# maxjiang93/space_time_pde

Measured on AMD Instinct MI355X. Metric: query-points/sec (fwd+PDE-residual bwd), rb2d 128^3 latent, higher is better.
Workload: dtype f32; 1 GPU; BASELINE configs[1]: latent [1,32,128,128,32], 2^20 query points, RB2 (3 transport + continuity), ImNet nf=32 softplus, L1 losses, backward to ImNet + UNet3d parameters; points=1048576, parallelism=points sharded x1, unet=UNet3d(igres=(32, 128, 128), nf=16, mf=256) fwd+bwd inside the timed step

## Files before the change

### include/stpde_hip.h

```cpp
#ifndef STPDE_HIP_H
#define STPDE_HIP_H

#ifdef __cplusplus
extern "C" {
#endif

#define STPDE_OK 0
#define STPDE_E_BADARG 1
#define STPDE_E_UNSUPPORTED 2
#define STPDE_E_LAUNCH 3

#define STPDE_ACT_TANH 0
#define STPDE_ACT_RELU 1
#define STPDE_ACT_SOFTPLUS 2
#define STPDE_ACT_ELU 3
#define STPDE_ACT_SWISH 4
#define STPDE_ACT_LEAKYRELU 5

#define STPDE_XT 3
#define STPDE_PBAR_SLOTS 64

typedef struct {
  int S1;
  int S2;
  int pair0[6];
  int pair1[6];
  int act;
  float act_param;
  int combo;
  float alpha[6];
} stpde_jet_cfg;

int stpde_version(void);
int stpde_last_error(char* buf, unsigned long n);
#define STPDE_TUNE_CONV3_LDS_OFF 0
#define STPDE_TUNE_CONV3_LDS_MINBLK 1
#define STPDE_TUNE_CONV3_LDS_GX 2
#define STPDE_TUNE_CONV_WGRAD_LDS_GX 3
#define STPDE_TUNE_CONV1_WGRAD_LDS_GX 4
#define STPDE_TUNE_COUNT 5
int stpde_tune(const char* name, int value);
int stpde_trace_enable(int on);
long stpde_trace_read(char* buf, unsigned long n);

typedef struct {
  int P, N, B, n0, n1, n2, C;
  int p_base;
  float lo_c[3], hi_c[3], cube[3];
  float alpha[6];
} stpde_gather_desc;
int stpde_lig_gather(const stpde_gather_desc* d, const float* pts, const float* latent, float* X, float* XR,
                     float* coef, int* cell, float* cw , void* stream);

typedef struct {
  int ntiles, KT, MT, first_hidden;
  stpde_jet_cfg cfg;
  int mfma_bf16;
  int packed;
  int det;
} stpde_layer_desc;
int stpde_jet_layer_fwd(const stpde_layer_desc* d, const float* in_pre, const float* X, const float* Wh_pack,
                        const float* Ws_pack, const float* tanc, const float* W0s_pack, const float* tanc0,
                        float* out_pre, const float* cw ,
                        const void* Wh_pack_bf16, float* z0, void* stream);

int stpde_jet_tail_fwd(const stpde_jet_cfg* cfg, int ntiles, int nf16, const float* in_pre2, const float* X,
                       const float* const* Wh_pack, const float* const* Ws_pack, const float* const* tanc,
                       float* const* out_pre, const float* cw, void* stream);

int stpde_jet_tail_fwd_p(const stpde_jet_cfg* cfg, int ntiles, int nf16, const float* in_pre2, const float* X,
                         const float* const* Wh_pack, const float* const* Ws_pack, const float* const* tanc,
                         float* const* out_pre, const float* cw, int packed, const void* const* Wh16_pack, void* stream);

int stpde_jet_tail_bwd(const stpde_jet_cfg* cfg, int ntiles, int nf16, const float* abar5, const float* const* WhT_pack,
                       const float* const* pre, float* const* abar_out, const float* cw, float* act_param_bar,
                       void* stream);

int stpde_jet_tail_bwd_p(const stpde_jet_cfg* cfg, int ntiles, int nf16, const float* abar5, const float* const* WhT_pack,
                         const float* const* pre, float* const* abar_out, const float* cw, float* act_param_bar, int packed,
                         const void* const* WhT16_pack, void* stream);

int stpde_jet_layer_bwd(const stpde_layer_desc* d, const float* abar_out, const float* WhT_pack, float* in_pre,
                        const float* X, const float* W0s_pack, const float* tanc0, float* abar0, const float* cw,
                        float* act_param_bar, const void* WhT_pack_bf16 ,
                        float* abar0_tan, const float* z0, void* stream);

int stpde_jet_layer_bwd_to(const stpde_layer_desc* d, const float* abar_out, const float* WhT_pack, const float* in_pre,
                           float* abar_in, const float* cw, float* act_param_bar, const void* WhT_pack_bf16, void* stream);

int stpde_jet_wgrad(const stpde_layer_desc* d, int SP, const float* abar_out, const float* in_pre, const float* X,
                    const float* tanc0, float* dW_aug, const float* cw, void* stream);

int stpde_jet_fc1_bwd_supported(const stpde_layer_desc* d);
int stpde_jet_fc1_bwd(const stpde_layer_desc* d, const float* abar1, const void* WhT_pack_bf16, const float* z0,
                      const float* tanc0, const float* cw, const float* X, float* abar0, float* abar0_tan, float* dW_aug,
                      float* act_param_bar, void* stream);

int stpde_lig_reduce_fwd(const stpde_jet_cfg* cfg, int S_mlp, int P, int n_out, const float* out_pre,
                         const float* coef, float* jets, long ldp, void* stream);
int stpde_lig_reduce_bwd(const stpde_jet_cfg* cfg, int S_mlp, int P, int n_out, const float* jets_bar, long ldp,
                         const float* coef, float* abar_out, void* stream);

int stpde_jet_tan0_reduce(int ntiles, int MT, const float* abar0_tan, float* dW_aug, int ldw, int det ,
                          void* stream);

typedef struct {
  int ntiles, nlayers, C, n1, n2;
  int MT[8];
  int SP[8];
  int packed[8];
  int S[8];
} stpde_xbar_desc;
int stpde_lig_xbar_scatter(const stpde_xbar_desc* d, const float* const* abar, const float* const* WsL_pack,
                           const int* cell, float* dlatent, void* stream);
int stpde_lig_xbar_rows(const stpde_xbar_desc* d, const float* const* abar, const float* const* WsL_pack,
                        float* xrows, void* stream);
int stpde_lig_dlatent_reduce(int B, int n0, int n1, int n2, int C, const float* xrows, const int* perm,
                             const int* start, float* dlatent, void* stream);

typedef struct {
  int nlayers;
  int cin, cout, nf16;
  int KT[8], MT[8];
  const float* Wh[8];
  const float* WhT[8];
  const float* Ws[8];
  const float* WsL[8];
  const float* tanc[8];
  const void* Wh16[8];
  const void* WhT16[8];
  int mfma_bf16;
  int packed_mask;
  long dw_off[8];
} stpde_imnet_plan;
typedef struct {
  float* X;
  float* XR;
  float* coef;
  float* cw;
  int* cell;
  float* pre[8];
  float* abar2x;
  float* abar3x;
  float* tan0;
  float* abar0;
  float* abar1x;
  float* abar0x;
  float* xrows;
  int* perm;
  int* start;
  void* sort_tmp;
  unsigned long sort_tmp_bytes;
  float* abar4x;
} stpde_lig_workspace;
#define STPDE_F_STASH 1
#define STPDE_F_VALUE_TILES 2
#define STPDE_F_FUSED_TAIL 4
#define STPDE_F_TAN0_ROWSUM 8
#define STPDE_F_DETERMINISTIC 16
#define STPDE_F_WGRAD 32
#define STPDE_F_WGRAD_FP32 64
#define STPDE_F_PHASE_A 128
#define STPDE_F_PHASE_B 256
#define STPDE_F_NO_FC1_FUSED 512
#define STPDE_F_DET 1024
int stpde_lig_imnet_jet_fwd(const stpde_imnet_plan* plan, const stpde_jet_cfg* cfg_mlp, const stpde_jet_cfg* cfg_out,
                            const stpde_gather_desc* gd, const float* pts, const float* latent,
                            const stpde_lig_workspace* ws, float* jets, long ldp, int flags, void* stream);
int stpde_lig_imnet_jet_bwd(const stpde_imnet_plan* plan, const stpde_jet_cfg* cfg_mlp, const stpde_jet_cfg* cfg_out,
                            const stpde_jet_cfg* cfg_val, const stpde_gather_desc* gd, const stpde_lig_workspace* ws,
                            const float* jets_bar, long ldp, float* dW_flat, float* dlatent, float* act_param_bar,
                            int flags, void* stream);
unsigned long stpde_lig_sort_tmp_bytes(int P, long n_nodes);
int stpde_lig_cell_sort(int P, long n_nodes, const int* cell, int* perm, int* start, void* tmp, unsigned long tmp_bytes,
                        void* stream);

typedef struct {
  int P, N, B, dim, C;
  int n[4];
  float lo_c[4], hi_c[4], cube[4];
} stpde_interp_desc;
int stpde_interp_fwd(const stpde_interp_desc* d, const float* grid, const float* pts, float* out ,
                     float* corner_values , float* weights ,
                     float* x_relative , void* stream);
int stpde_interp_bwd_grid(const stpde_interp_desc* d, const float* pts, const float* out_bar,
                          const float* corner_bar, float* dgrid, void* stream);

typedef struct {
  int D, P, N, B, C;
  int p_base;
  int ntiles;
  int n[4];
  float lo_c[4], hi_c[4], cube[4];
// ... 222 lines not shown
```

### space_time_pde_amd/csrc/api.cpp

```cpp
#include <hip/hip_runtime.h>

#include <cstdarg>
#include <cstdio>
#include <cstring>
#include <mutex>
#include <set>
#include <string>

#include "../../include/stpde_hip.h"

static thread_local char g_err[512] = "";

void stpde_set_error(const char* fmt, ...) {
  va_list ap;
  va_start(ap, fmt);
  vsnprintf(g_err, sizeof(g_err), fmt, ap);
  va_end(ap);
}

int stpde_check_launch(const char* what) {
  hipError_t e = hipGetLastError();
  if (e != hipSuccess) {
    stpde_set_error("%s: launch failed: %s", what, hipGetErrorString(e));
    return STPDE_E_LAUNCH;
  }
  return STPDE_OK;
}

extern "C" int stpde_version(void) { return 316; }

#include <atomic>
static const char* const g_tune_names[STPDE_TUNE_COUNT] = {"conv3_lds_off", "conv3_lds_minblk", "conv3_lds_gx", "conv_wgrad_lds_gx",
                                                           "conv1_wgrad_lds_gx"};
static std::atomic<int> g_tune[STPDE_TUNE_COUNT];
int stpde_tune_get(int key) { return (key >= 0 && key < STPDE_TUNE_COUNT) ? g_tune[key].load(std::memory_order_relaxed) : 0; }
extern "C" int stpde_tune(const char* name, int value) {
  if (!name) return -1;
  for (int k = 0; k < STPDE_TUNE_COUNT; ++k)
    if (!strcmp(name, g_tune_names[k])) return g_tune[k].exchange(value);
  stpde_set_error("stpde_tune: unknown key '%s'", name);
  return -1;
}

extern "C" int stpde_last_error(char* buf, unsigned long n) {
  if (!buf || n == 0) return STPDE_E_BADARG;
  strncpy(buf, g_err, n - 1);
  buf[n - 1] = 0;
  return STPDE_OK;
}

int stpde_trace_on = 0;
static std::mutex g_trace_mu;
static std::set<std::string> g_trace;

void stpde_trace_note(const char* launcher, const char* kernel) {
  std::lock_guard<std::mutex> lk(g_trace_mu);
  g_trace.insert(std::string(kernel) + " @ " + launcher);
}

extern "C" int stpde_trace_enable(int on) {
  std::lock_guard<std::mutex> lk(g_trace_mu);
  g_trace.clear();
  stpde_trace_on = on ? 1 : 0;
  return STPDE_OK;
}

extern "C" long stpde_trace_read(char* buf, unsigned long n) {
  std::lock_guard<std::mutex> lk(g_trace_mu);
  std::string all;
  for (const auto& s : g_trace) all += s + "\n";
  if (buf && n > 0) {
    strncpy(buf, all.c_str(), n - 1);
    buf[n - 1] = 0;
  }
  return (long)all.size() + 1;
}
```

### space_time_pde_amd/csrc/jet_wgrad_impl.h

```cpp
#pragma once
#include <cstdlib>

#include "common.h"

struct WgradArgs {
  const float* P;
  const float* Q;
  const float* X;
  const float* tanc0;
  float* dW;
  const float* cw;
  int SP, KT, MT, ntiles;
  int gx, gy, gz;
  int kz0;
  int det;
  int bf16;
  int pk;
  int ncoord;
  int xfold;
  stpde_jet_cfg cfg;
};

#ifndef STPDE_QUAD_PIPE
#define STPDE_QUAD_PIPE 1
#endif
#ifndef STPDE_ABLATE_W
#define STPDE_ABLATE_W 0
#endif
#ifndef STPDE_X3_XFOLD
#define STPDE_X3_XFOLD 1
#endif
#ifndef STPDE_WG_RPIPE
#define STPDE_WG_RPIPE 1
#endif
#ifndef STPDE_X3_EARLYP
#define STPDE_X3_EARLYP 0
#endif
template <int TP>
__device__ __forceinline__ void lds_put_T(float* blk, int lane, f32x4 v) {
  const int g = lane >> 4, j = lane & 15;
  float* w = blk + (4 * g) * TP + j;
  w[0] = v[0];
  w[TP] = v[1];
  w[2 * TP] = v[2];
  w[3 * TP] = v[3];
}
template <int TP>
__device__ __forceinline__ void lds_put_R(float* blk, int lane, f32x4 v) {
  *reinterpret_cast<f32x4*>(blk + (lane & 15) * TP + 4 * (lane >> 4)) = v;
}
template <int TP>
__device__ __forceinline__ f32x4 lds_get_R(const float* blk, int lane) {
  return *reinterpret_cast<const f32x4*>(blk + (lane & 15) * TP + 4 * (lane >> 4));
}

template <int S1, int S2, int MODE, int ACT, int KC, bool HASX, bool BF = false, int SPL = 1, int PKM = 0>
__global__ __launch_bounds__(512, 2) void k_wgrad_coop(WgradArgs a) {
  static_assert(SPL == 1 || (BF && SPL == 3), "operand splitting is a bf16-pipe mode");
  constexpr int PMODE = (PKM & 4) ? 2 : 0;
  constexpr int S = 1 + S1 + S2, MCW = 2, NW = 8, RS = 8;
  constexpr int NM = KC;
  constexpr bool SPLP = BF && SPL == 3;
  constexpr int TP = (2 * RS * S * 16 * 24 * 4 + NW * 2 * 16 * 24 * 4 <= 150 * 1024) ? 24 : 20;
  constexpr int TBLK = 16 * TP;
  constexpr int BLK = BF ? 128 * SPL : TBLK;
  constexpr int NBUF = (2 * RS * S * BLK * 4 + NW * 2 * BLK * 4 <= 150 * 1024) ? 2 : 1;
  constexpr int SX = S1 == 3 ? 4 : 1;
  __shared__ __attribute__((aligned(16))) float hl[NBUF][RS][S][BLK];
  constexpr int NPP = (BF && SPL == 1 && 2 * RS * S * 512 + NW * S * MCW * 512 <= 100 * 1024) ? S * MCW : 2;
  __shared__ __attribute__((aligned(16))) float pp[NW][NPP][BLK];
  const int lane = threadIdx.x & 63;
  const int wv = threadIdx.x >> 6;
  const int lo = lane * 4;
  const int KT = a.KT, MT = a.MT, SP = a.SP;
  const int L = blockIdx.x, xcd = L & 7, slot = L >> 3;
  const int kz = (slot % a.gz) + a.kz0, tq = slot / a.gz;
  const int mg = tq % a.gy, bx = (tq / a.gy) * 8 + xcd;
  const int ms = wv % NM, ks = wv / NM;
  const int mt0 = (mg * NM + ms) * MCW;
  const int kq0 = kz * RS;
  const int g = lane >> 4, c = lane & 15;

  f32x4 acc[MCW][KC];
#pragma unroll
  for (int mi = 0; mi < MCW; ++mi)
#pragma unroll
    for (int ki = 0; ki < KC; ++ki) acc[mi][ki] = f32x4{0.f, 0.f, 0.f, 0.f};

  auto put = [&](float* blk, f32x4 v, bool row_major) {
    if constexpr (BF) {
      __bf16* hb16 = reinterpret_cast<__bf16*>(blk);
#pragma unroll
      for (int t = 0; t < SPL; ++t) {
        const bf16x4 h = to_bf4(v);
        *reinterpret_cast<bf16x4*>(hb16 + (t * 16 + (lane & 15)) * 16 + 4 * (lane >> 4)) = h;
        if (t + 1 < SPL) v -= bf4_to_f32(h);
      }
    } else if (row_major) {
      lds_put_R<TP>(blk, lane, v);
    } else {
      lds_put_T<TP>(blk, lane, v);
    }
  };
  auto get = [&](const float* blk) -> f32x4 { return lds_get_R<TP>(blk, lane); };
  auto get16 = [&](const float* blk, int t, bool cm = true) -> bf16x4 {
    const __bf16* b16 = reinterpret_cast<const __bf16*>(blk) + t * 256;
    if (cm) return lds_read_tr16(b16 + (4 * (lane >> 4) + ((lane & 15) >> 2)) * 16 + 4 * (lane & 3));
    return *reinterpret_cast<const bf16x4*>(b16 + (lane & 15) * 16 + 4 * (lane >> 4));
  };

  auto x_rowmajor = [&](f32x4 v) -> f32x4 {
    float* patch = pp[wv][0];
    __builtin_amdgcn_wave_barrier();
    lds_put_T<TP>(patch, lane, v);
    __builtin_amdgcn_wave_barrier();
    const f32x4 r = lds_get_R<TP>(patch, lane);
    __builtin_amdgcn_wave_barrier();
    return r;
  };
  auto x_rowmajor16 = [&](f32x4 v, bf16x4* t) {
    float* patch = pp[wv][0];
    __builtin_amdgcn_wave_barrier();
    put(patch, v, false);
    __builtin_amdgcn_wave_barrier();
#pragma unroll
    for (int k = 0; k < (BF ? SPL : 1); ++k) t[k] = get16(patch, k, true);
    __builtin_amdgcn_wave_barrier();
  };
  auto load_q = [&](int tile, f32x4* pre, float* cq) {
    const int kq = kq0 + wv;
    if (!HASX || kq < KT) {
      load_cq<S2>(a.cw, tile * 2 + (c >> 3), cq);
      if (MODE == 1) {
        pre[0] = ld4(a.Q + ((size_t)tile * KT + kq) * 256 + lo);
        if (S1 == 3) {
#pragma unroll
          for (int d = 0; d < 3; ++d) pre[1 + d] = ld4(a.tanc0 + ((size_t)d * KT + kq) * 256 + lo);
#pragma unroll
          for (int p = 0; p < S2; ++p) pre[4 + p] = f32x4{0.f, 0.f, 0.f, 0.f};
        }
      } else {
#pragma unroll
        for (int st = 0; st < S; ++st) pre[st] = ld_blk(a.Q, (PKM & 1) ? 1 : 0, tile, S, KT, st, kq, lane);
      }
    } else if (kq < KT + XT) {
      pre[0] = ld4(a.X + ((size_t)tile * XT + (kq - KT)) * 256 + lo);
    }
  };
  auto finish_q = [&](const f32x4* pre, const float* cq, int buf) {
    const int kq = kq0 + wv;
    if (!HASX || kq < KT) {
      f32x4 H[S];
      act_jet_fwd<S1, S2, ACT>(a.cfg, pre, H, cq);
#pragma unroll
      for (int st = 0; st < S; ++st) put(&hl[buf][wv][st][0], H[st], false);
    } else if (kq < KT + XT) {
      const int xt = kq - KT;
      put(&hl[buf][wv][0][0], pre[0], false);
      if (S1 == 3) {
#pragma unroll
        for (int d = 0; d < 3; ++d) {
          f32x4 v;
#pragma unroll
          for (int r = 0; r < 4; ++r) v[r] = (xt == 0 && 4 * g + r == d && d < a.ncoord) ? 1.f : 0.f;
          put(&hl[buf][wv][1 + d][0], v, false);
        }
      }
    }
  };
  auto produce = [&](int tile, int buf) {
    f32x4 pre[S];
    float cq[6];
// ... 4 lines not shown
#pragma unroll
    for (int st = 0; st < S; ++st)
#pragma unroll
      for (int mi = 0; mi < MCW; ++mi) {
        const int mt = mt0 + mi < MT ? mt0 + mi : MT - 1;
        raw[st][mi] = st < SP ? ld_blk_raw(a.P, PMODE, tile, SP, MT, st, mt, lane) : f32x4{0.f, 0.f, 0.f, 0.f};
      }
  };
  auto transpose_p = [&](f32x4 (*raw)[MCW], f32x4 (*pa)[MCW]) {
    if constexpr (BF) return;
#pragma unroll
    for (int st = 0; st < S; ++st)
#pragma unroll
      for (int mi = 0; mi < MCW; ++mi) {
        float* patch = pp[wv][(st * MCW + mi) & 1];
        lds_put_T<TP>(patch, lane, blk_val(raw[st][mi], st < SP ? PMODE : 0, st));
        __builtin_amdgcn_wave_barrier();
        pa[st][mi] = lds_get_R<TP>(patch, lane);
        __builtin_amdgcn_wave_barrier();
      }
  };

  constexpr int SH = (S + 1) / 2, SXH = (SX + 1) / 2;
  bf16x8 pa8[BF ? SPL : 1][BF ? SH : 1][MCW];
  const bf16x4 zero4 = to_bf4(f32x4{0.f, 0.f, 0.f, 0.f});
  auto pack_p = [&](f32x4 (*raw_)[MCW]) {
    if constexpr (BF && NPP > 2) {
#pragma unroll
      for (int st = 0; st < S; ++st)
#pragma unroll
        for (int mi = 0; mi < MCW; ++mi) put(pp[wv][st * MCW + mi], blk_val(raw_[st][mi], st < SP ? PMODE : 0, st), false);
      __builtin_amdgcn_wave_barrier();
#pragma unroll
      for (int sp = 0; sp < SH; ++sp)
#pragma unroll
        for (int mi = 0; mi < MCW; ++mi)
          pa8[0][sp][mi] = cat8(get16(pp[wv][2 * sp * MCW + mi], 0, true),
                                2 * sp + 1 < S ? get16(pp[wv][(2 * sp + 1 < S ? 2 * sp + 1 : 0) * MCW + mi], 0, true) : zero4);
      __builtin_amdgcn_wave_barrier();
    } else if constexpr (BF) {
      int flip = 0;
      auto terms = [&](f32x4 v, bf16x4* t) {
        float* patch = pp[wv][flip];
        flip ^= 1;
        put(patch, v, false);
        __builtin_amdgcn_wave_barrier();
#pragma unroll
        for (int k = 0; k < SPL; ++k) t[k] = get16(patch, k, true);
        __builtin_amdgcn_wave_barrier();
      };
#pragma unroll
      for (int sp = 0; sp < SH; ++sp)
#pragma unroll
        for (int mi = 0; mi < MCW; ++mi) {
          bf16x4 t0[SPL], t1[SPL];
          terms(blk_val(raw_[2 * sp][mi], 2 * sp < SP ? PMODE : 0, 2 * sp), t0);
          if (2 * sp + 1 < S) terms(blk_val(raw_[2 * sp + 1][mi], 2 * sp + 1 < SP ? PMODE : 0, 2 * sp + 1), t1);
#pragma unroll
          for (int k = 0; k < SPL; ++k) pa8[k][sp][mi] = cat8(t0[k], 2 * sp + 1 < S ? t1[k] : zero4);
        }
    }
  };
  auto mma16 = [&](f32x4& c, int sp, int mi, const bf16x8* H8) {
    if constexpr (SPL == 3) {
      constexpr int TP[6] = {1, 0, 2, 0, 1, 0}, TH[6] = {1, 2, 0, 1, 0, 0};
#pragma unroll
      for (int q6 = 0; q6 < 6; ++q6) c = mfma_bf(pa8[TP[q6]][sp][mi], H8[TH[q6]], c);
    } else {
      c = mfma_bf(pa8[0][sp][mi], H8[0], c);
    }
  };

  const int stride = a.gx;
  int tile = bx;
  f32x4 pa[S][MCW];
  constexpr bool XF = !HASX && !BF;
  constexpr bool XB = !HASX && BF && SPL == 1;
  constexpr bool XS = !HASX && BF && SPL == 3 && STPDE_X3_XFOLD;
  const int xslot = (kz - a.kz0) * (NW / NM) + ks;
  const int xsel = xslot < XT ? xslot : XT - 1;
  f32x4 accx[(XF || XB || XS) ? MCW : 1];
  float acct[XF && S1 == 3 ? 3 : 1][XF ? MCW : 1];
  const bf16x4 one4 = to_bf4(f32x4{1.f, 1.f, 1.f, 1.f});
  const bool tanw = (XB || XS) && S1 == 3 && xslot == 0;
  const bf16x4 e0 = (tanw && c == 0) ? one4 : zero4;
  const bf16x8 x8t = cat8((tanw && c == 1 && a.ncoord > 1) ? one4 : zero4, (tanw && c == 2 && a.ncoord > 2) ? one4 : zero4);
  f32x4 xr = f32x4{0.f, 0.f, 0.f, 0.f};
  if constexpr (XF || XB || XS) {
#pragma unroll
    for (int mi = 0; mi < MCW; ++mi) accx[mi] = f32x4{0.f, 0.f, 0.f, 0.f};
  }
  if constexpr (XF && S1 == 3) {
#pragma unroll
    for (int d = 0; d < 3; ++d)
#pragma unroll
      for (int mi = 0; mi < MCW; ++mi) acct[d][mi] = 0.f;
  }
  auto xb_mma = [&]() {
    if constexpr (XB) {
      bf16x4 xt1[1];
      x_rowmajor16(xr, xt1);
      const bf16x8 x8 = cat8(xt1[0], S1 == 3 ? e0 : zero4);
#pragma unroll
      for (int mi = 0; mi < MCW; ++mi) accx[mi] = mfma_bf(pa8[0][0][mi], x8, accx[mi]);
      if constexpr (S1 == 3) {
#pragma unroll
        for (int mi = 0; mi < MCW; ++mi) accx[mi] = mfma_bf(pa8[0][1][mi], x8t, accx[mi]);
      }
    }
  };
  auto xs_mma = [&]() {
    if constexpr (XS) {
      bf16x4 xt3[3];
      x_rowmajor16(xr, xt3);
      constexpr int TP[6] = {1, 0, 2, 0, 1, 0}, TH[6] = {1, 2, 0, 1, 0, 0};
#pragma unroll
      for (int q6 = 0; q6 < 6; ++q6) {
        const bf16x8 x8 = cat8(xt3[TH[q6]], (S1 == 3 && TH[q6] == 0) ? e0 : zero4);
#pragma unroll
        for (int mi = 0; mi < MCW; ++mi) accx[mi] = mfma_bf(pa8[TP[q6]][0][mi], x8, accx[mi]);
      }
      if constexpr (S1 == 3) {
#pragma unroll
        for (int k = 2; k >= 0; --k)
#pragma unroll
          for (int mi = 0; mi < MCW; ++mi) accx[mi] = mfma_bf(pa8[k][1][mi], x8t, accx[mi]);
      }
    }
  };
  auto ring_mma = [&](int rb) {
    auto rd = [&](int ki, bf16x8* H8) {
      const int q = ks * KC + ki;
#pragma unroll
      for (int sp = 0; sp < SH; ++sp)
        H8[sp] = cat8(get16(&hl[rb][q][2 * sp][0], 0, true),
                      2 * sp + 1 < S ? get16(&hl[rb][q][2 * sp + 1 < S ? 2 * sp + 1 : 0][0], 0, true) : zero4);
    };
    bf16x8 Hn[SH];
    rd(0, Hn);
#pragma unroll
    for (int ki = 0; ki < KC; ++ki) {
      bf16x8 Hc[SH];
#pragma unroll
      for (int sp = 0; sp < SH; ++sp) Hc[sp] = Hn[sp];
      if (ki + 1 < KC) rd(ki + 1, Hn);
      __builtin_amdgcn_sched_barrier(0);
#pragma unroll
      for (int sp = 0; sp < SH; ++sp)
#pragma unroll
        for (int mi = 0; mi < MCW; ++mi) acc[mi][ki] = mfma_bf(pa8[0][sp][mi], Hc[sp], acc[mi][ki]);
      __builtin_amdgcn_sched_barrier(0);
    }
  };
  if (tile < a.ntiles) {
    f32x4 raw[S][MCW];
    produce(tile, 0);
    load_p_raw(tile, raw);
    transpose_p(raw, pa);
    pack_p(raw);
    if constexpr (XF || XB || XS) {
      if (a.xfold) xr = ld4(a.X + ((size_t)tile * XT + xsel) * 256 + lo);
    }
  }
  __syncthreads();
  __builtin_amdgcn_s_waitcnt(0x0F70);
  int buf = 0;
  constexpr bool SWAPOK = BF && SPL == 1 && NBUF == 2 && !HASX && PKM != 0 && MODE == 1;
  if constexpr (SWAPOK) {
    if (wv >= NW / 2) {
      auto pack_to = [&](f32x4 (*raw_)[MCW], bf16x8 (*dst)[MCW]) {
        if constexpr (NPP > 2) {
#pragma unroll
          for (int st = 0; st < S; ++st)
#pragma unroll
            for (int mi = 0; mi < MCW; ++mi) put(pp[wv][st * MCW + mi], blk_val(raw_[st][mi], st < SP ? PMODE : 0, st), false);
          __builtin_amdgcn_wave_barrier();
#pragma unroll
          for (int sp = 0; sp < SH; ++sp)
#pragma unroll
            for (int mi = 0; mi < MCW; ++mi)
              dst[sp][mi] = cat8(get16(pp[wv][2 * sp * MCW + mi], 0, true),
                                 2 * sp + 1 < S ? get16(pp[wv][(2 * sp + 1 < S ? 2 * sp + 1 : 0) * MCW + mi], 0, true) : zero4);
          __builtin_amdgcn_wave_barrier();
          return;
        }
        int flip = 0;
        auto term = [&](f32x4 v) -> bf16x4 {
          float* patch = pp[wv][flip];
          flip ^= 1;
          put(patch, v, false);
          __builtin_amdgcn_wave_barrier();
          const bf16x4 t = get16(patch, 0, true);
          __builtin_amdgcn_wave_barrier();
          return t;
        };
#pragma unroll
        for (int sp = 0; sp < SH; ++sp)
#pragma unroll
          for (int mi = 0; mi < MCW; ++mi) {
            const bf16x4 t0 = term(blk_val(raw_[2 * sp][mi], 2 * sp < SP ? PMODE : 0, 2 * sp));
            bf16x4 t1 = zero4;
            if (2 * sp + 1 < S) t1 = term(blk_val(raw_[2 * sp + 1][mi], 2 * sp + 1 < SP ? PMODE : 0, 2 * sp + 1));
            dst[sp][mi] = cat8(t0, t1);
          }
      };
      f32x4 raw[S][MCW];
      f32x4 preq[S];
      float cqq[6];
      f32x4 xrn = f32x4{0.f, 0.f, 0.f, 0.f};
      if (tile < a.ntiles) {
        const int nx0 = tile + stride < a.ntiles ? tile + stride : tile;
        load_p_raw(nx0, raw);
        load_q(nx0, preq, cqq);
        if constexpr (XB) xrn = ld4(a.X + ((size_t)nx0 * XT + xsel) * 256 + lo);
      }
      for (; tile < a.ntiles; tile += stride) {
        const int next = tile + stride;
        const int nx = next < a.ntiles ? next : tile;
        bf16x8 tmp8[SH][MCW];
        finish_q(preq, cqq, buf ^ 1);
        pack_to(raw, tmp8);
        const f32x4 xr_next = xrn;
        const int nn = nx + stride < a.ntiles ? nx + stride : nx;
        load_p_raw(nn, raw);
        load_q(nn, preq, cqq);
        if constexpr (XB) xrn = ld4(a.X + ((size_t)nn * XT + xsel) * 256 + lo);
        xb_mma();
        ring_mma(buf);
#pragma unroll
        for (int sp = 0; sp < SH; ++sp)
#pragma unroll
          for (int mi = 0; mi < MCW; ++mi) pa8[0][sp][mi] = tmp8[sp][mi];
        if constexpr (XB) xr = xr_next;
        __syncthreads();
        buf ^= 1;
      }
    }
  }
  for (; tile < a.ntiles; tile += stride) {
    const int next = tile + stride;
    const int nx = next < a.ntiles ? next : tile;
    f32x4 raw[S][MCW];
    constexpr bool EARLYP = S < 8 && !(XS && !STPDE_X3_EARLYP);
    if (EARLYP) load_p_raw(nx, raw);
    f32x4 preq[S];
    float cqq[6];
    constexpr bool EARLYQ = BF && SPL == 1;
    if (EARLYQ && NBUF == 2 && STPDE_ABLATE_W != 3) load_q(nx, preq, cqq);
    constexpr bool EARLYZ = !BF && MODE == 1 && !HASX && NBUF == 2;
    f32x4 z0e = f32x4{0.f, 0.f, 0.f, 0.f};
    if constexpr (EARLYZ) z0e = ld4(a.Q + ((size_t)nx * KT + kq0 + wv) * 256 + lo);
    f32x4 xrn = f32x4{0.f, 0.f, 0.f, 0.f};
    if constexpr (XB) {
      xrn = ld4(a.X + ((size_t)nx * XT + xsel) * 256 + lo);
      xb_mma();
    }
    if constexpr (XS) {
      xrn = ld4(a.X + ((size_t)nx * XT + xsel) * 256 + lo);
      xs_mma();
    }
    if constexpr (XF) {
      xrn = ld4(a.X + ((size_t)nx * XT + xsel) * 256 + lo);
      const f32x4 xrr = x_rowmajor(xr);
#pragma unroll
      for (int mi = 0; mi < MCW; ++mi)
#pragma unroll
        for (int r = 0; r < 4; ++r) accx[mi] = mfma4(pa[0][mi][r], xrr[r], accx[mi]);
      if constexpr (S1 == 3) {
#pragma unroll
        for (int d = 0; d < 3; ++d)
#pragma unroll
          for (int mi = 0; mi < MCW; ++mi)
            acct[d][mi] += (pa[1 + d][mi][0] + pa[1 + d][mi][1]) + (pa[1 + d][mi][2] + pa[1 + d][mi][3]);
      }
    }
    if constexpr (SPLP && !HASX && KC % 2 == 0) {
#pragma unroll
      for (int ki = 0; ki < KC; ki += 2) {
        const int q = ks * KC + ki;
#pragma unroll
        for (int sp = 0; sp < SH; ++sp) {
          bf16x8 H8[2][3];
#pragma unroll
          for (int kk = 0; kk < 2; ++kk)
#pragma unroll
            for (int k = 0; k < 3; ++k)
              H8[kk][k] = STPDE_ABLATE_W == 4 ? pa8[k][sp][kk] :
                          cat8(get16(&hl[buf][q + kk][2 * sp][0], k),
                               2 * sp + 1 < S ? get16(&hl[buf][q + kk][2 * sp + 1 < S ? 2 * sp + 1 : 0][0], k) : zero4);
          constexpr int TP[6] = {1, 0, 2, 0, 1, 0}, TH[6] = {1, 2, 0, 1, 0, 0};
#pragma unroll
          for (int q6 = (STPDE_ABLATE_W == 1 ? 5 : 0); q6 < 6; ++q6)
#pragma unroll
            for (int kk = 0; kk < 2; ++kk)
#pragma unroll
              for (int mi = 0; mi < MCW; ++mi)
                acc[mi][ki + kk] = mfma_bf(pa8[TP[q6]][sp][mi], H8[kk][TH[q6]], acc[mi][ki + kk]);
        }
      }
    } else if constexpr (BF && SPL == 1 && !HASX && STPDE_ABLATE_W == 0) {
      ring_mma(buf);
    } else if constexpr (!BF && !HASX && STPDE_WG_RPIPE) {
      constexpr int PIN = 0x2 | 0x4 | 0x10 | 0x20 | 0x40 | 0x200;
      f32x4 Hc = get(&hl[buf][ks * KC][0][0]);
#pragma unroll
      for (int ki = 0; ki < KC; ++ki) {
        const int q = ks * KC + ki;
#pragma unroll
        for (int st = 0; st < S; ++st) {
          f32x4 Hn = Hc;
          if (st + 1 < S) Hn = get(&hl[buf][q][st + 1][0]);
          else if (ki + 1 < KC) Hn = get(&hl[buf][q + 1][0][0]);
          __builtin_amdgcn_sched_barrier(PIN);
#pragma unroll
          for (int r = 0; r < 4; ++r)
#pragma unroll
            for (int mi = 0; mi < MCW; ++mi) acc[mi][ki] = mfma4(pa[st][mi][r], Hc[r], acc[mi][ki]);
          __builtin_amdgcn_sched_barrier(PIN);
          Hc = Hn;
        }
      }
    } else {
#pragma unroll
    for (int ki = 0; ki < KC; ++ki) {
      const int q = ks * KC + ki;
      const int kq = kq0 + q;
      if (!HASX || kq < KT) {
        f32x4 H[S];
        if constexpr (!BF) {
#pragma unroll
          for (int st = 0; st < S; ++st) H[st] = get(&hl[buf][q][st][0]);
        }
        if constexpr (BF) {
#pragma unroll
          for (int sp = 0; sp < SH; ++sp) {
            bf16x4 t0[SPL], t1[SPL];
            bf16x8 H8[SPL];
#pragma unroll
            for (int k = 0; k < SPL; ++k) {
              t0[k] = get16(&hl[buf][q][2 * sp][0], k, true);
              if (2 * sp + 1 < S) t1[k] = get16(&hl[buf][q][2 * sp + 1 < S ? 2 * sp + 1 : 0][0], k, true);
            }
#pragma unroll
            for (int k = 0; k < SPL; ++k) H8[k] = cat8(t0[k], 2 * sp + 1 < S ? t1[k] : zero4);
#pragma unroll
            for (int mi = 0; mi < MCW; ++mi) mma16(acc[mi][ki], sp, mi, H8);
          }
        } else {
#pragma unroll
        for (int mi = 0; mi < MCW; ++mi)
#pragma unroll
          for (int r = 0; r < 4; ++r)
#pragma unroll
            for (int st = 0; st < S; ++st) acc[mi][ki] = mfma4(pa[st][mi][r], H[st][r], acc[mi][ki]);
        }
      } else if (kq < KT + XT) {
        f32x4 H[SX];
        if constexpr (!BF) {
#pragma unroll
          for (int st = 0; st < SX; ++st) H[st] = get(&hl[buf][q][st][0]);
        }
        if constexpr (BF) {
#pragma unroll
          for (int sp = 0; sp < SXH; ++sp) {
            bf16x4 t0[SPL], t1[SPL];
            bf16x8 H8[SPL];
#pragma unroll
            for (int k = 0; k < SPL; ++k) {
              t0[k] = get16(&hl[buf][q][2 * sp][0], k, true);
              if (2 * sp + 1 < SX) t1[k] = get16(&hl[buf][q][2 * sp + 1 < SX ? 2 * sp + 1 : 0][0], k, true);
            }
#pragma unroll
            for (int k = 0; k < SPL; ++k) H8[k] = cat8(t0[k], 2 * sp + 1 < SX ? t1[k] : zero4);
#pragma unroll
            for (int mi = 0; mi < MCW; ++mi) mma16(acc[mi][ki], sp, mi, H8);
          }
        } else {
#pragma unroll
        for (int mi = 0; mi < MCW; ++mi)
#pragma unroll
          for (int r = 0; r < 4; ++r)
#pragma unroll
            for (int st = 0; st < SX; ++st) acc[mi][ki] = mfma4(pa[st][mi][r], H[st][r], acc[mi][ki]);
        }
      }
    }
    }
    if constexpr (XF || XB || XS) xr = xrn;
    if (NBUF == 2) {
      if (STPDE_ABLATE_W != 3) {
        if constexpr (EARLYZ) __builtin_amdgcn_sched_barrier(0);
        if (!EARLYQ) load_q(nx, preq, cqq);
        if constexpr (EARLYZ) preq[0] = z0e;
        finish_q(preq, cqq, buf ^ 1);
      }
      if (!EARLYP) load_p_raw(nx, raw);
      if (STPDE_ABLATE_W != 2) {
        transpose_p(raw, pa);
        pack_p(raw);
      }
      if (STPDE_ABLATE_W != 5) __syncthreads();
      buf ^= 1;
    } else {
      __syncthreads();
      produce(nx, 0);
      if (!EARLYP) load_p_raw(nx, raw);
      transpose_p(raw, pa);
      pack_p(raw);
      __syncthreads();
    }
  }

  const int ldw = 16 * (KT + XT);
#pragma unroll
  for (int mi = 0; mi < MCW; ++mi) {
    const int mt = mt0 + mi;
    if (mt >= MT) continue;
#pragma unroll
    for (int ki = 0; ki < KC; ++ki) {
      const int kq = kq0 + ks * KC + ki;
      if (kq >= KT + XT) continue;
#pragma unroll
      for (int r = 0; r < 4; ++r)
        acc_add_f32(a.dW, (size_t)(16 * mt + 4 * g + r) * ldw + 16 * kq + c, acc[mi][ki][r], a.det);
    }
  }
  if constexpr (XB || XS) {
    if (a.xfold && xslot < XT) {
#pragma unroll
      for (int mi = 0; mi < MCW; ++mi) {
        const int mt = mt0 + mi;
        if (mt >= MT) continue;
#pragma unroll
        for (int r = 0; r < 4; ++r)
          acc_add_f32(a.dW, (size_t)(16 * mt + 4 * g + r) * ldw + 16 * (KT + xslot) + c, accx[mi][r], a.det);
      }
    }
  }
  if constexpr (XF) {
    if (a.xfold && xslot < XT) {
#pragma unroll
      for (int mi = 0; mi < MCW; ++mi) {
        const int mt = mt0 + mi;
        if (mt >= MT) continue;
#pragma unroll
        for (int r = 0; r < 4; ++r)
          acc_add_f32(a.dW, (size_t)(16 * mt + 4 * g + r) * ldw + 16 * (KT + xslot) + c, accx[mi][r], a.det);
        if constexpr (S1 == 3) {
          if (xslot == 0) {
#pragma unroll
            for (int d = 0; d < 3; ++d) {
              float v = acct[d][mi];
              v += __shfl_xor(v, 16, 64);
              v += __shfl_xor(v, 32, 64);
              if (g == 0 && d < a.ncoord) acc_add_f32(a.dW, (size_t)(16 * mt + c) * ldw + 16 * KT + d, v, a.det);
            }
          }
        }
      }
    }
  }
}

template <int S1, int S2, int ACT, int MCW, int KTT, int PKW = 0, bool BFM = false>
__global__ __launch_bounds__(256, (MCW * (KTT + XT) <= 8) ? 3 : ((MCW * (KTT + XT) <= 14) ? 2 : 1)) void k_wgrad_wave(WgradArgs a) {
  constexpr int S = 1 + S1 + S2, NK = KTT + XT;
  constexpr int TP = 24, TBLK = 16 * TP;
  __shared__ __attribute__((aligned(16))) float pp[4][2][TBLK];
  const int lane = threadIdx.x & 63;
  const int wv = threadIdx.x >> 6;
  const int lo = lane * 4;
  const int MT = a.MT;
  const int mt0 = blockIdx.y * MCW;
  const int g = lane >> 4, c = lane & 15;
// ... 302 lines not shown
#pragma unroll
  for (int mi = 0; mi < MCW; ++mi)
#pragma unroll
    for (int k = 0; k <= KW; ++k) acc[mi][k] = f32x4{0.f, 0.f, 0.f, 0.f};
  float2 praw[S];
  f32x4 qraw[KW][S];
  f32x4 xr = f32x4{0.f, 0.f, 0.f, 0.f};
  auto load_p = [&](int t) {
    const char* pb = reinterpret_cast<const char*>(a.P) + (size_t)t * (S * MCW * 512) + (size_t)wv * 512 + lane * 8;
#pragma unroll
    for (int st = 0; st < S; ++st) praw[st] = *reinterpret_cast<const float2*>(pb + (size_t)st * MCW * 512);
    if (wv < XT) xr = ld4(a.X + ((size_t)t * XT + wv) * 256 + lo);
  };
  auto load_qk = [&](int t, int k) {
#pragma unroll
    for (int st = 0; st < S; ++st) qraw[k][st] = ld_blk_raw(a.Q, 1, t, S, KTT, st, KW * wv + k, lane);
  };
  if ((int)blockIdx.x < a.ntiles) {
    load_p(blockIdx.x);
#pragma unroll
    for (int k = 0; k < KW; ++k) load_qk(blockIdx.x, k);
  }
#pragma unroll 1
  for (int tile = blockIdx.x; tile < a.ntiles; tile += gridDim.x) {
    const int tnext = tile + (int)gridDim.x < a.ntiles ? tile + (int)gridDim.x : tile;
    float cq[6];
    load_cq<S2>(a.cw, tile * 2 + (c >> 3), cq);
#pragma unroll
    for (int st = 0; st < S; ++st) *reinterpret_cast<float2*>(&pshare[st][wv][wofs]) = praw[st];
    f32x4 xcur = xr;
    if (wv < XT) {
      float* patch = reinterpret_cast<float*>(&ppriv[wv][0][0][0]);
      lds_put_T<20>(patch, lane, xr);
      __builtin_amdgcn_wave_barrier();
      xcur = lds_get_R<20>(patch, lane);
      __builtin_amdgcn_wave_barrier();
    }
    load_p(tnext);
#pragma unroll
    for (int k = 0; k < KW; ++k) {
      f32x4 pre[S], H[S];
#pragma unroll
      for (int st = 0; st < S; ++st) pre[st] = blk_val(qraw[k][st], 1, st);
      load_qk(tnext, k);
      act_jet_fwd<S1, S2, ACT>(a.cfg, pre, H, cq);
#pragma unroll
      for (int st = 0; st < S; ++st) *reinterpret_cast<bf16x4*>(&ppriv[wv][k][st][wofs]) = to_bf4(H[st]);
    }
    __syncthreads();
    bf16x4 h16[KW][S];
#pragma unroll
    for (int k = 0; k < KW; ++k)
#pragma unroll
      for (int st = 0; st < S; ++st) h16[k][st] = lds_read_tr16(&ppriv[wv][k][st][rofs]);
#pragma unroll
    for (int st = 0; st < S; ++st) {
#pragma unroll
      for (int mi = 0; mi < MCW; ++mi) {
        const bf16x4 pa = lds_read_tr16(&pshare[st][mi][rofs]);
#pragma unroll
        for (int k = 0; k < KW; ++k) acc[mi][k] = mfma_bf16k(pa, h16[k][st], acc[mi][k]);
        if (st == 0) {
          if (wv < XT) {
            const f32x4 p0 = bf4_to_f32(pa);
#pragma unroll
            for (int r = 0; r < 4; ++r) acc[mi][KW] = mfma4(p0[r], xcur[r], acc[mi][KW]);
          }
        } else if (st <= 3) {
          if (wv == 0) acc[mi][KW] = mfma_bf16k(pa, c == st - 1 ? one4 : zero4, acc[mi][KW]);
        }
      }
    }
    __syncthreads();
  }
  const int ldw = 16 * (KTT + XT);
#pragma unroll
  for (int mi = 0; mi < MCW; ++mi) {
#pragma unroll
    for (int k = 0; k <= KW; ++k) {
      if (k == KW && wv >= XT) continue;
      const int col = k < KW ? 16 * (KW * wv + k) : 16 * (KTT + wv);
#pragma unroll
      for (int r = 0; r < 4; ++r) acc_add_f32(a.dW, (size_t)(16 * mi + 4 * g + r) * ldw + col + c, acc[mi][k][r], a.det);
    }
  }
}

template <int S1, int S2, int ACT, int MCW, int KTT>
static int launch_wgrad_wave(const WgradArgs& a, hipStream_t stream) {
  const int gy = (a.MT + MCW - 1) / MCW;
  int gx = 768 / gy;
  if (gx > (a.ntiles + 3) / 4) gx = (a.ntiles + 3) / 4;
  if (gx < 1) gx = 1;
  if (a.pk) {
    if constexpr (S1 == 3 && ((KTT == 8 && (MCW == 4 || MCW == 2)) || (KTT == 4 && MCW == 2) || (KTT == 2 && MCW == 1))) {
      if (a.pk == 5) {
        STPDE_LAUNCH((k_wgrad_wave<S1, S2, ACT, MCW, KTT, 3, true>), dim3(gx, gy), dim3(256), 0, stream, a);
        return stpde_check_launch("k_wgrad_wave");
      }
      if (a.pk == 1) {
        STPDE_LAUNCH((k_wgrad_wave<S1, S2, ACT, MCW, KTT, 1, true>), dim3(gx, gy), dim3(256), 0, stream, a);
        return stpde_check_launch("k_wgrad_wave");
      }
    }
    stpde_set_error("jet_wgrad: packed operands (%d) not compiled for this narrow-layer shape", a.pk);
    return STPDE_E_UNSUPPORTED;
  }
  STPDE_LAUNCH((k_wgrad_wave<S1, S2, ACT, MCW, KTT>), dim3(gx, gy), dim3(256), 0, stream, a);
  return stpde_check_launch("k_wgrad_wave");
}

template <int S1, int S2, int ACT>
static int try_wgrad_wave(const WgradArgs& a, hipStream_t stream) {
  if (a.MT > 4 || a.SP != 1 + S1 + S2 || a.bf16) return -1;
  if constexpr (S1 + S2 > 5) {
    return -1;
  } else {
    if (a.MT == 1) {
      if (a.KT == 2) return launch_wgrad_wave<S1, S2, ACT, 1, 2>(a, stream);
      if (a.KT == 4) return launch_wgrad_wave<S1, S2, ACT, 1, 4>(a, stream);
    } else {
      if (a.KT == 2) return launch_wgrad_wave<S1, S2, ACT, 2, 2>(a, stream);
      if (a.KT == 4) return launch_wgrad_wave<S1, S2, ACT, 2, 4>(a, stream);
      if constexpr (S1 == 3) {
        if (a.KT == 8 && a.MT == 4 && XT == 3 && (a.pk == 0 || a.pk == 5)) {
          int gx = 768;
          if (gx > a.ntiles) gx = a.ntiles;
          if (a.pk) {
            STPDE_LAUNCH((k_wgrad_oct_bf<S1, S2, ACT, 4>), dim3(gx), dim3(256), 0, stream, a);
            return stpde_check_launch("k_wgrad_oct_bf");
          }
          STPDE_LAUNCH((k_wgrad_quad<S1, S2, ACT, 0, false>), dim3(gx), dim3(256), 0, stream, a);
          return stpde_check_launch("k_wgrad_quad");
        }
      }
      if (a.KT == 8 && a.MT == 4) return launch_wgrad_wave<S1, S2, ACT, 4, 8>(a, stream);
      if (a.KT == 8) return launch_wgrad_wave<S1, S2, ACT, 2, 8>(a, stream);
    }
    return -1;
  }
}

template <int S1, int S2, int MODE, int ACT, int KC>
static int launch_wgrad_kc(const WgradArgs& a0, hipStream_t stream) {
  WgradArgs a = a0;
  if (a.KT == 0 && a.pk == 4 && a.bf16 == 1) a.pk = 5;
  a.gy = (a.MT + 2 * KC - 1) / (2 * KC);
  const int ngr = (a.KT + XT + 7) / 8;
  const int nhid = a.KT / 8;
  const int kslots = 8 / KC;
  constexpr bool SPLIT_OK = KC >= 4 && S1 + S2 <= 4;
  const int bfm = (a.bf16 == 3 && !SPLIT_OK) ? 0 : a.bf16;
  const bool xfold = (!bfm || (bfm == 1 && KC >= 4) || (bfm == 3 && KC >= 4 && STPDE_X3_XFOLD)) && a.KT > 0 && a.KT % 8 == 0 && nhid * kslots >= XT && a.X;
  for (int part = 0; part < 2; ++part) {
    a.kz0 = part == 0 ? 0 : nhid;
    a.gz = part == 0 ? nhid : ngr - nhid;
    a.xfold = (xfold && part == 0) ? 1 : 0;
    if (a.gz <= 0 || (xfold && part == 1)) continue;
    int gx = 512 / (a.gy * a.gz);
    if (gx > a.ntiles) gx = a.ntiles;
    gx = (gx + 7) / 8 * 8;
    if (gx < 8) gx = 8;
    a.gx = gx;
    constexpr bool HAS_BF = KC >= 4;
    const dim3 grid(gx * a.gy * a.gz);
    if (HAS_BF && bfm == 3) {
      if constexpr (SPLIT_OK) {
        if (part == 0)
          STPDE_LAUNCH((k_wgrad_coop<S1, S2, MODE, ACT, KC, false, true, 3>), grid, dim3(512), 0, stream, a);
        else
          STPDE_LAUNCH((k_wgrad_coop<S1, S2, MODE, ACT, KC, true, true, 3>), grid, dim3(512), 0, stream, a);
      }
    } else if (HAS_BF && bfm) {
      if constexpr (HAS_BF) {
        constexpr int PKA = MODE == 1 ? 4 : 5;
        if (a.pk != 0 && a.pk != PKA) {
          stpde_set_error("packed layer buffers: combination %d not compiled for this weight-gradient kind", a.pk);
          return STPDE_E_UNSUPPORTED;
        }
        if (part == 0 && a.pk)
          STPDE_LAUNCH((k_wgrad_coop<S1, S2, MODE, ACT, KC, false, true, 1, PKA>), grid, dim3(512), 0, stream, a);
        else if (part == 0)
          STPDE_LAUNCH((k_wgrad_coop<S1, S2, MODE, ACT, KC, false, true>), grid, dim3(512), 0, stream, a);
        else if (a.pk)
          STPDE_LAUNCH((k_wgrad_coop<S1, S2, MODE, ACT, KC, true, true, 1, PKA>), grid, dim3(512), 0, stream, a);
        else
          STPDE_LAUNCH((k_wgrad_coop<S1, S2, MODE, ACT, KC, true, true>), grid, dim3(512), 0, stream, a);
      }
    } else if (a.pk) {
      if constexpr (S1 == 0 && S2 == 0 && MODE == 0 && KC == 8) {
        if (a.pk == 4 && part != 0) {
          STPDE_LAUNCH((k_wgrad_coop<S1, S2, MODE, ACT, KC, true, false, 1, 4>), grid, dim3(512), 0, stream, a);
          int rc = stpde_check_launch("k_wgrad_coop");
          if (rc) return rc;
          continue;
        }
      }
      stpde_set_error("packed layer buffers: combination %d not compiled for the fp32 weight-gradient kernels", a.pk);
      return STPDE_E_UNSUPPORTED;
    } else if (part == 0) {
      STPDE_LAUNCH((k_wgrad_coop<S1, S2, MODE, ACT, KC, false>), grid, dim3(512), 0, stream, a);
    } else {
      STPDE_LAUNCH((k_wgrad_coop<S1, S2, MODE, ACT, KC, true>), grid, dim3(512), 0, stream, a);
    }
    int rc = stpde_check_launch("k_wgrad_coop");
    if (rc) return rc;
  }
  return STPDE_OK;
}

template <int S1, int S2, int MODE, int ACT>
static int launch_wgrad_act(const WgradArgs& a, hipStream_t stream) {
  if constexpr (MODE == 0) {
    const int rc = try_wgrad_wave<S1, S2, ACT>(a, stream);
    if (rc >= 0) return rc;
    if constexpr (S1 == 3 && S1 + S2 <= 5) {
      if (a.KT == 16 && a.MT == 8 && XT == 3 && a.SP == 1 + S1 + S2 && a.X &&
          ((a.bf16 == 0 && a.pk == 0) || (a.bf16 == 1 && a.pk == 5) || (a.bf16 == 3 && a.pk == 0))) {
        int gx = 256;
        if (gx > a.ntiles) gx = a.ntiles;
        if (a.pk) {
          STPDE_LAUNCH((k_wgrad_oct_bf<S1, S2, ACT>), dim3(gx), dim3(512), 0, stream, a);
          return stpde_check_launch("k_wgrad_oct_bf");
        }
        STPDE_LAUNCH((k_wgrad_quad<S1, S2, ACT, 0, false, 8>), dim3(gx), dim3(512), 0, stream, a);
        return stpde_check_launch("k_wgrad_quad");
      }
    }
  }
  if (a.MT >= 16) return launch_wgrad_kc<S1, S2, MODE, ACT, 8>(a, stream);
  if constexpr (MODE == 1) {
    return launch_wgrad_kc<S1, S2, MODE, ACT, 4>(a, stream);
  } else {
    if (a.MT >= 8) return launch_wgrad_kc<S1, S2, MODE, ACT, 4>(a, stream);
    if (a.MT >= 4) return launch_wgrad_kc<S1, S2, MODE, ACT, 2>(a, stream);
    return launch_wgrad_kc<S1, S2, MODE, ACT, 1>(a, stream);
  }
}

template <int S1, int S2>
static int launch_mode(const WgradArgs& a, int mode, hipStream_t stream) {
  if (mode == 0) {
    switch (a.cfg.act) {
      case STPDE_ACT_TANH: return launch_wgrad_act<S1, S2, 0, STPDE_ACT_TANH>(a, stream);
      case STPDE_ACT_RELU: return launch_wgrad_act<S1, S2, 0, STPDE_ACT_RELU>(a, stream);
      case STPDE_ACT_SOFTPLUS: return launch_wgrad_act<S1, S2, 0, STPDE_ACT_SOFTPLUS>(a, stream);
      case STPDE_ACT_ELU: return launch_wgrad_act<S1, S2, 0, STPDE_ACT_ELU>(a, stream);
      case STPDE_ACT_LEAKYRELU: return launch_wgrad_act<S1, S2, 0, STPDE_ACT_LEAKYRELU>(a, stream);
      default: return launch_wgrad_act<S1, S2, 0, STPDE_ACT_SWISH>(a, stream);
    }
  }
  switch (a.cfg.act) {
    case STPDE_ACT_TANH: return launch_wgrad_act<S1, S2, 1, STPDE_ACT_TANH>(a, stream);
    case STPDE_ACT_RELU: return launch_wgrad_act<S1, S2, 1, STPDE_ACT_RELU>(a, stream);
    case STPDE_ACT_SOFTPLUS: return launch_wgrad_act<S1, S2, 1, STPDE_ACT_SOFTPLUS>(a, stream);
    case STPDE_ACT_ELU: return launch_wgrad_act<S1, S2, 1, STPDE_ACT_ELU>(a, stream);
    case STPDE_ACT_LEAKYRELU: return launch_wgrad_act<S1, S2, 1, STPDE_ACT_LEAKYRELU>(a, stream);
    default: return launch_wgrad_act<S1, S2, 1, STPDE_ACT_SWISH>(a, stream);
  }
}

#define STPDE_DEFINE_WGRAD_TU(S1, S2) \
  int stpde_wgrad_launch_##S1##_##S2(const WgradArgs& a, int mode, hipStream_t stream) { return launch_mode<S1, S2>(a, mode, stream); }

int stpde_wgrad_launch_0_0(const WgradArgs& a, int mode, hipStream_t stream);
int stpde_wgrad_launch_3_0(const WgradArgs& a, int mode, hipStream_t stream);
int stpde_wgrad_launch_3_1(const WgradArgs& a, int mode, hipStream_t stream);
int stpde_wgrad_launch_3_2(const WgradArgs& a, int mode, hipStream_t stream);
int stpde_wgrad_launch_3_4(const WgradArgs& a, int mode, hipStream_t stream);
int stpde_wgrad_launch_3_6(const WgradArgs& a, int mode, hipStream_t stream);
```

Measured before the change: 2.501 million query-points/s.

## Add wave-split software pipeline for FP32 wgrad with interleaved P prefetch

Adds an FP32 weight-gradient main loop that splits the workgroup's waves into early and late halves, which stagger the Q-tile staging into LDS. The next tile's P operands are loaded from global memory piecewise, interleaved between the MFMA steps of the ring product. This is meant to hide global-load latency behind matrix math and to spread LDS staging across waves. The path is on by default when SP matches 1+S1+S2 (the tune key only disables it with value 2). In exchange it raises register pressure from the extra prefetch buffers and shifts the order of loads and barriers, and it refactors the existing fold and ring loops into shared lambdas.

```diff
diff --git a/include/stpde_hip.h b/include/stpde_hip.h
--- a/include/stpde_hip.h
+++ b/include/stpde_hip.h
@@ -38,7 +38,8 @@
 #define STPDE_TUNE_CONV3_LDS_GX 2
 #define STPDE_TUNE_CONV_WGRAD_LDS_GX 3
 #define STPDE_TUNE_CONV1_WGRAD_LDS_GX 4
-#define STPDE_TUNE_COUNT 5
+#define STPDE_TUNE_WGRAD_FP32_SWAP 5
+#define STPDE_TUNE_COUNT 6
 int stpde_tune(const char* name, int value);
 int stpde_trace_enable(int on);
 long stpde_trace_read(char* buf, unsigned long n);
diff --git a/space_time_pde_amd/csrc/api.cpp b/space_time_pde_amd/csrc/api.cpp
--- a/space_time_pde_amd/csrc/api.cpp
+++ b/space_time_pde_amd/csrc/api.cpp
@@ -31,7 +31,7 @@
 
 #include <atomic>
 static const char* const g_tune_names[STPDE_TUNE_COUNT] = {"conv3_lds_off", "conv3_lds_minblk", "conv3_lds_gx", "conv_wgrad_lds_gx",
-                                                           "conv1_wgrad_lds_gx"};
+                                                           "conv1_wgrad_lds_gx", "wgrad_fp32_swap"};
 static std::atomic<int> g_tune[STPDE_TUNE_COUNT];
 int stpde_tune_get(int key) { return (key >= 0 && key < STPDE_TUNE_COUNT) ? g_tune[key].load(std::memory_order_relaxed) : 0; }
 extern "C" int stpde_tune(const char* name, int value) {
diff --git a/space_time_pde_amd/csrc/jet_wgrad_impl.h b/space_time_pde_amd/csrc/jet_wgrad_impl.h
--- a/space_time_pde_amd/csrc/jet_wgrad_impl.h
+++ b/space_time_pde_amd/csrc/jet_wgrad_impl.h
@@ -18,6 +18,7 @@
   int pk;
   int ncoord;
   int xfold;
+  int swap;
   stpde_jet_cfg cfg;
 };
 
@@ -328,6 +329,47 @@
       __builtin_amdgcn_sched_barrier(0);
     }
   };
+  auto xf_fold = [&]() {
+    if constexpr (XF) {
+      const f32x4 xrr = x_rowmajor(xr);
+#pragma unroll
+      for (int mi = 0; mi < MCW; ++mi)
+#pragma unroll
+        for (int r = 0; r < 4; ++r) accx[mi] = mfma4(pa[0][mi][r], xrr[r], accx[mi]);
+      if constexpr (S1 == 3) {
+#pragma unroll
+        for (int d = 0; d < 3; ++d)
+#pragma unroll
+          for (int mi = 0; mi < MCW; ++mi)
+            acct[d][mi] += (pa[1 + d][mi][0] + pa[1 + d][mi][1]) + (pa[1 + d][mi][2] + pa[1 + d][mi][3]);
+      }
+    }
+  };
+  constexpr int PIN_MFMA_DSR = 0x2 | 0x4 | 0x10 | 0x20 | 0x40 | 0x200;
+  constexpr int PIN_MFMA_DSR_VMEM = 0x2 | 0x4 | 0x200;
+  auto ring_mma32 = [&](int rb, auto pin_c, auto&& side) {
+    constexpr int PIN = decltype(pin_c)::value;
+    f32x4 Hc = get(&hl[rb][ks * KC][0][0]);
+#pragma unroll
+    for (int ki = 0; ki < KC; ++ki) {
+      const int q = ks * KC + ki;
+#pragma unroll
+      for (int st = 0; st < S; ++st) {
+        f32x4 Hn = Hc;
+        if (st + 1 < S) Hn = get(&hl[rb][q][st + 1][0]);
+        else if (ki + 1 < KC) Hn = get(&hl[rb][q + 1][0][0]);
+        __builtin_amdgcn_sched_barrier(PIN);
+        side(ki * S + st);
+#pragma unroll
+        for (int r = 0; r < 4; ++r)
+#pragma unroll
+          for (int mi = 0; mi < MCW; ++mi) acc[mi][ki] = mfma4(pa[st][mi][r], Hc[r], acc[mi][ki]);
+        __builtin_amdgcn_sched_barrier(PIN);
+        Hc = Hn;
+      }
+    }
+  };
+  auto no_side = [](int) {};
   if (tile < a.ntiles) {
     f32x4 raw[S][MCW];
     produce(tile, 0);
@@ -409,6 +451,60 @@
           for (int mi = 0; mi < MCW; ++mi) pa8[0][sp][mi] = tmp8[sp][mi];
         if constexpr (XB) xr = xr_next;
         __syncthreads();
+        buf ^= 1;
+      }
+    }
+  }
+  constexpr bool SWAP32 = !BF && SPL == 1 && PKM == 0 && MODE == 1 && !HASX && NBUF == 2 && S <= 5 && STPDE_WG_RPIPE;
+  if constexpr (SWAP32) {
+    if (a.swap) {
+      const bool late = wv >= NW / 2;
+      const int rmo = (c >> 2) * 64 + 16 * g + (c & 3);
+      const int mtc0 = mt0 < MT ? mt0 : MT - 1, mtc1 = mt0 + 1 < MT ? mt0 + 1 : MT - 1;
+      f32x4 pn[S][MCW];
+      f32x4 z0n = f32x4{0.f, 0.f, 0.f, 0.f}, xrn = f32x4{0.f, 0.f, 0.f, 0.f};
+      if (late && tile < a.ntiles)
+        z0n = ld4(a.Q + ((size_t)(tile + stride < a.ntiles ? tile + stride : tile) * KT + kq0 + wv) * 256 + lo);
+      auto prep = [&](int t) {
+        if (STPDE_ABLATE_W != 3) {
+          f32x4 preq[S];
+          float cqq[6];
+          load_q(t, preq, cqq);
+          preq[0] = z0n;
+          finish_q(preq, cqq, buf ^ 1);
+        }
+      };
+      for (; tile < a.ntiles; tile += stride) {
+        const int next = tile + stride;
+        const int nx = next < a.ntiles ? next : tile;
+        const int nn = nx + stride < a.ntiles ? nx + stride : nx;
+        if (late) prep(nx);
+        __builtin_amdgcn_sched_barrier(0);
+        z0n = ld4(a.Q + ((size_t)(late ? nn : nx) * KT + kq0 + wv) * 256 + lo);
+        xrn = ld4(a.X + ((size_t)nx * XT + xsel) * 256 + lo);
+        const float* pb = a.P + (size_t)nx * S * MT * 256 + rmo;
+        __builtin_amdgcn_sched_barrier(0);
+        xf_fold();
+        ring_mma32(buf, std::integral_constant<int, PIN_MFMA_DSR_VMEM>{}, [&](int n) {
+          constexpr int DPB = (MCW * 4 + KC - 1) / KC;
+          if (STPDE_ABLATE_W != 2) {
+#pragma unroll
+            for (int e = n * DPB; e < (n + 1) * DPB && e < S * MCW * 4; ++e) {
+              const int st = e / (4 * MCW), mi = (e / 4) % MCW, r = e % 4;
+              pn[st][mi][r] = pb[((size_t)st * MT + (mi ? mtc1 : mtc0)) * 256 + 4 * r];
+            }
+          }
+        });
+        __builtin_amdgcn_sched_barrier(0);
+        if (!late) prep(nx);
+        if (STPDE_ABLATE_W != 2) {
+#pragma unroll
+          for (int st = 0; st < S; ++st)
+#pragma unroll
+            for (int mi = 0; mi < MCW; ++mi) pa[st][mi] = pn[st][mi];
+        }
+        xr = xrn;
+        if (STPDE_ABLATE_W != 5) __syncthreads();
         buf ^= 1;
       }
     }
@@ -437,18 +533,7 @@
     }
     if constexpr (XF) {
       xrn = ld4(a.X + ((size_t)nx * XT + xsel) * 256 + lo);
-      const f32x4 xrr = x_rowmajor(xr);
-#pragma unroll
-      for (int mi = 0; mi < MCW; ++mi)
-#pragma unroll
-        for (int r = 0; r < 4; ++r) accx[mi] = mfma4(pa[0][mi][r], xrr[r], accx[mi]);
-      if constexpr (S1 == 3) {
-#pragma unroll
-        for (int d = 0; d < 3; ++d)
-#pragma unroll
-          for (int mi = 0; mi < MCW; ++mi)
-            acct[d][mi] += (pa[1 + d][mi][0] + pa[1 + d][mi][1]) + (pa[1 + d][mi][2] + pa[1 + d][mi][3]);
-      }
+      xf_fold();
     }
     if constexpr (SPLP && !HASX && KC % 2 == 0) {
 #pragma unroll
@@ -477,25 +562,7 @@
     } else if constexpr (BF && SPL == 1 && !HASX && STPDE_ABLATE_W == 0) {
       ring_mma(buf);
     } else if constexpr (!BF && !HASX && STPDE_WG_RPIPE) {
-      constexpr int PIN = 0x2 | 0x4 | 0x10 | 0x20 | 0x40 | 0x200;
-      f32x4 Hc = get(&hl[buf][ks * KC][0][0]);
-#pragma unroll
-      for (int ki = 0; ki < KC; ++ki) {
-        const int q = ks * KC + ki;
-#pragma unroll
-        for (int st = 0; st < S; ++st) {
-          f32x4 Hn = Hc;
-          if (st + 1 < S) Hn = get(&hl[buf][q][st + 1][0]);
-          else if (ki + 1 < KC) Hn = get(&hl[buf][q + 1][0][0]);
-          __builtin_amdgcn_sched_barrier(PIN);
-#pragma unroll
-          for (int r = 0; r < 4; ++r)
-#pragma unroll
-            for (int mi = 0; mi < MCW; ++mi) acc[mi][ki] = mfma4(pa[st][mi][r], Hc[r], acc[mi][ki]);
-          __builtin_amdgcn_sched_barrier(PIN);
-          Hc = Hn;
-        }
-      }
+      ring_mma32(buf, std::integral_constant<int, PIN_MFMA_DSR>{}, no_side);
     } else {
 #pragma unroll
     for (int ki = 0; ki < KC; ++ki) {
@@ -1104,6 +1171,7 @@
   constexpr bool SPLIT_OK = KC >= 4 && S1 + S2 <= 4;
   const int bfm = (a.bf16 == 3 && !SPLIT_OK) ? 0 : a.bf16;
   const bool xfold = (!bfm || (bfm == 1 && KC >= 4) || (bfm == 3 && KC >= 4 && STPDE_X3_XFOLD)) && a.KT > 0 && a.KT % 8 == 0 && nhid * kslots >= XT && a.X;
+  a.swap = (stpde_tune_get(STPDE_TUNE_WGRAD_FP32_SWAP) != 2 && a.SP == 1 + S1 + S2) ? 1 : 0;
   for (int part = 0; part < 2; ++part) {
     a.kz0 = part == 0 ? 0 : nhid;
     a.gz = part == 0 ? nhid : ngr - nhid;
```

New measurement: 2.533 million query-points/s (median of 6 runs). 1.01x the previous value.
